# FitSNAP/FitSNAP

Measured on AMD Instinct MI355X. Metric: training rows/sec through A^T A + solve, 1000000 x 128 fp64 in total over the GPUs (strong scaling), higher is better.
Workload: dtype f64

## Files before the change

fitsnap_amd/build.py:

```python
from __future__ import annotations

import hashlib
import os
import shutil
import subprocess
import sys

HERE = os.path.dirname(os.path.abspath(__file__))
CSRC = os.path.join(HERE, "csrc")
LIBDIR = os.path.join(HERE, "_lib")
LIBNAME = "libfsnap_hip.so"
SOURCES = ["fsnap_syrk_quad.hip:0", "fsnap_syrk_quad.hip:1", "fsnap_syrk_quad.hip:2", "fsnap_syrk.hip", "fsnap_syrk_short.hip", "fsnap_rows.hip", "fsnap_chol.hip", "fsnap_trsm.hip", "fsnap_fused.hip", "fsnap_merr.hip", "fsnap_cand.hip", "fsnap_uq.hip", "fsnap_loco.hip", "fsnap_mcmc.hip", "fsnap_capi.cpp", "fsnap_comm.cpp", "fsnap_p2p.cpp",
           "fsnap_rowspace.cpp", "fsnap_rowspace_host.cpp", "fsnap_solve.cpp"]
HEADERS = ["fsnap_kernels.h", "fsnap_device_common.h", "fsnap_ctx.h", "fsnap_rowspace_host.h", "fsnap_condest.h", "fsnap_p2p.h", os.path.join("..", "..", "include", "fsnap_hip.h")]
ARCH = "gfx950"


def lib_path() -> str:
    return os.path.join(LIBDIR, LIBNAME)


def _hipcc() -> str:
    exe = shutil.which("hipcc") or "/opt/rocm/bin/hipcc"
    if not os.path.exists(exe):
        raise RuntimeError("hipcc not found: libfsnap_hip.so cannot be built")
    return exe


def _source_digest() -> str:
    h = hashlib.sha256()
    for name in sorted({s.split(":")[0] for s in SOURCES}) + HEADERS:
        with open(os.path.join(CSRC, name), "rb") as f:
            h.update(f.read())
    return h.hexdigest()


def build_library(force: bool = False, verbose: bool = False) -> str:
    os.makedirs(LIBDIR, exist_ok=True)
    out = lib_path()
    stamp = out + ".sha256"
    digest = _source_digest()
    if not force and os.path.exists(out) and os.path.exists(stamp):
        with open(stamp) as f:
            if f.read().strip() == digest:
                return out
    hipcc = _hipcc()
    objs = []
    common = [f"--offload-arch={ARCH}", "-O3", "-std=c++17", "-fPIC", "-I", os.path.join(HERE, "..", "include")]
    procs = []
    objdir = os.path.join(LIBDIR, "obj")
    os.makedirs(objdir, exist_ok=True)
    hh = hashlib.sha256()
    for name in HEADERS:
        with open(os.path.join(CSRC, name), "rb") as f:
            hh.update(f.read())
    for entry in SOURCES:
        src, _, part = entry.partition(":")
        obj = os.path.join(objdir, os.path.splitext(src)[0] + (f"_{part}" if part else "") + ".o")
        cmd = [hipcc, *common]
        if part:
            cmd += [f"-DFSNAP_QUAD_PART={part}"]
        if src in ("fsnap_capi.cpp", "fsnap_comm.cpp", "fsnap_p2p.cpp", "fsnap_rowspace.cpp"):
            cmd += ["-x", "hip"]
        if src in ("fsnap_solve.cpp", "fsnap_rowspace_host.cpp"):
            cmd = [hipcc, "-x", "c++", "-O3", "-std=c++17", "-fPIC", "-mavx2", "-mfma",
# ... 39 lines not shown
```

fitsnap_amd/csrc/fsnap_capi.cpp:

```cpp
#include <hip/hip_runtime.h>

#include <algorithm>
#include <atomic>
#include <chrono>
#include <cstdarg>
#include <cstdio>
#include <cstdlib>
#include <cstring>
#include <limits>
#include <new>
#include <queue>
#include <string>
#include <thread>
#include <vector>

#include "../../include/fsnap_hip.h"
#include "fsnap_kernels.h"

extern "C" int fsnap_solve_diag_tagged(int kind, double param, int64_t K, const double* G, const double* c, const double* diag,
                                       double* beta, int* rank, double* rcond_est, int upper, const void* owner,
                                       unsigned long long generation);
extern "C" int fsnap_solve_diag_upper(int kind, double param, int64_t K, const double* G, const double* c, const double* diag,
                                      double* beta, int* rank, double* rcond_est);
extern "C" int fsnap_solve_diag(int kind, double param, int64_t K, const double* G, const double* c, const double* diag,
// ... 523 lines not shown
    a.nblocks = g.nblocks;
    a.split = g.split;
    a.chunks_per_wave = g.cpw;
    a.nontemporal = true;
    a.part = (double*)ctx->part.p;
    a.cpart = (double*)ctx->cpart.p;
    a.spart = (double*)ctx->spart.p;
    int ns = -1;
    const double* spart_src = a.spart;
    if (g.fused_pack) {
        a.fused_pack = true;
    } else {
        int npk = 0;
        if ((rc = ensure_wpack(ctx, &npk))) return rc;
        a.wpack = ctx->wpack_override ? ctx->wpack_override : (const double*)ctx->wpack.p;
        spart_src = (const double*)ctx->wpack_spart.p;
        ns = npk;
    }
    hipEvent_t* evs;
    if ((rc = fit_events(ctx, &evs))) return rc;
    if (evs) FSNAP_HIP(hipEventRecord(evs[0], ctx->stream), "hipEventRecord");
    if (g.quad && g.cluster > 1) {
        const size_t need = (size_t)g.nblocks * 4 * sizeof(int);
        if (ctx->quad_flow.bytes < need) {
            if (!ctx->quad_flow.ensure(need)) return ctx->fail(FSNAP_E_NOMEM, "hipMalloc(flow words) failed");
            FSNAP_HIP(hipMemsetAsync(ctx->quad_flow.p, 0, ctx->quad_flow.bytes, ctx->stream), "hipMemset(flow words)");
            ctx->quad_flow_tag = 0;
        }
        ctx->quad_flow_tag += 1u << 20;
        a.flow_words = (int*)ctx->quad_flow.p;
        const int flow = 2 | ((g.cluster == 2 ? 0 : 2) << 2);
        a.flow_tag = (int)(ctx->quad_flow_tag | (unsigned)flow);
    }
    if (g.shortk) FSNAP_HIP(fsnap::launch_syrk_short(a, ctx->stream), "launch fsnap_syrk_short");
    else if (g.quad) FSNAP_HIP(fsnap::launch_syrk_quad(a, ctx->stream), "launch fsnap_syrk_quad");
    else if (g.acc) FSNAP_HIP(fsnap::launch_syrk_acc(a, ctx->stream), "launch fsnap_syrk_acc");
    else FSNAP_HIP(fsnap::launch_syrk_wave_p(a, ctx->stream), "launch fsnap_syrk_wave_p");
    if (evs) FSNAP_HIP(hipEventRecord(evs[1], ctx->stream), "hipEventRecord");
    double* mirror = nullptr;
    if (want_mirror && !device_factor(ctx, ctx->K)) {
        const size_t need = ((size_t)FSNAP_PACKED_LEN(ctx->K) + (size_t)ctx->K) * 8;
        if (ctx->mirror_bytes < need) {
            if (ctx->mirror) (void)hipHostFree(ctx->mirror);
            ctx->mirror = nullptr;
            ctx->mirror_bytes = 0;
            if (hipHostMalloc((void**)&ctx->mirror, need, hipHostMallocCoherent | hipHostMallocMapped) == hipSuccess)
                ctx->mirror_bytes = need;
        }
        if (ctx->mirror && !ctx->mirror_ev && hipEventCreateWithFlags(&ctx->mirror_ev, hipEventDisableTiming) != hipSuccess)
            ctx->mirror_ev = nullptr;
        if (ctx->mirror && ctx->mirror_ev) mirror = ctx->mirror;
    }
    const bool upper_mirror = mirror != nullptr;
    FSNAP_HIP(fsnap::launch_reduce(a.part, a.cpart, spart_src, g.nblocks, cs_per_block, ns, a.K, d_packed, mirror, accumulate,
                                   ctx->stream, upper_mirror),
              "launch fsnap_reduce_partials");
    if (evs) FSNAP_HIP(hipEventRecord(evs[2], ctx->stream), "hipEventRecord");
    if (mirror) {
        FSNAP_HIP(hipEventRecord(ctx->mirror_ev, ctx->stream), "hipEventRecord");
        ctx->mirror_of = d_packed;
        ctx->mirror_K = ctx->K;
        ctx->mirror_upper = upper_mirror;
        ctx->mirror_gen = next_mirror_generation();
    }
    if (evs) ctx->t_syrk = true;
    return FSNAP_OK;
}

}

namespace fsnap {

int wpack_current(fsnap_ctx* ctx) {
    int rc, npk = 0;
    if ((rc = check_rows(ctx)) || (rc = check_weights(ctx))) return rc;
    return ensure_wpack(ctx, &npk);
}

int normal_eq_launch_on(fsnap_ctx* ctx, const double* Q, int64_t ldq, const double* qpack, double* d_packed) {
    const double* const save_A = ctx->dA;
    const int64_t save_lda = ctx->lda;
    ctx->dA = Q;
    ctx->lda = ldq;
    ctx->wpack_override = qpack;
    const int rc = launch_normal_eq(ctx, d_packed);
    ctx->wpack_override = nullptr;
    ctx->dA = save_A;
    ctx->lda = save_lda;
    return rc;
}

}

extern "C" {

int fsnap_version(void) { return 200; }

int fsnap_device_count(int* count) {
    if (!count) return FSNAP_E_ARG;
    int n = 0;
    hipError_t e = hipGetDeviceCount(&n);
    if (e != hipSuccess) {
        g_last_error = std::string("hipGetDeviceCount: ") + hipGetErrorString(e);
        *count = 0;
        return FSNAP_E_HIP;
    }
    *count = n;
    return FSNAP_OK;
}
// ... 86 lines not shown

int fsnap_ctx_set_stream(fsnap_ctx* ctx, void* hip_stream) {
    if (!ctx) return FSNAP_E_ARG;
    FSNAP_HIP(hipStreamSynchronize(ctx->stream), "hipStreamSynchronize");
    ctx->stream = (hipStream_t)hip_stream;
    return FSNAP_OK;
}

int fsnap_ctx_use_own_stream(fsnap_ctx* ctx) {
    if (!ctx) return FSNAP_E_ARG;
    FSNAP_HIP(hipStreamSynchronize(ctx->stream), "hipStreamSynchronize");
    ctx->stream = ctx->own_stream;
    return FSNAP_OK;
}

int fsnap_set_option(fsnap_ctx* ctx, const char* key, int64_t value) {
    if (!ctx || !key) return FSNAP_E_ARG;
    if (!strcmp(key, "device_solve")) {
        if (value < 0 || value > 2) return ctx->fail(FSNAP_E_ARG, "device_solve must be 0 (auto), 1 (always) or 2 (never)");
        ctx->opt_device_solve = (int)value;
    } else if (!strcmp(key, "tiled")) {
        ctx->opt_tiled = value != 0;
    } else if (!strcmp(key, "short")) {
        if (value < -1 || value > 1) return ctx->fail(FSNAP_E_ARG, "short must be -1 (by the row count), 0 (never) or 1 (always)");
        ctx->opt_short = (int)value;
    } else if (!strcmp(key, "timing_every")) {
        if (value < 0 || value > (1 << 20)) return ctx->fail(FSNAP_E_ARG, "timing_every out of range");
        ctx->opt_timing_every = (int)value;
        ctx->timing_phase = 0;
    } else if (!strcmp(key, "repack")) {
        ctx->opt_repack = value != 0;
    } else if (!strcmp(key, "comm_timeout")) {
        if (value < 0 || value > 86400) return ctx->fail(FSNAP_E_ARG, "comm_timeout must be 0 (FSNAP_COMM_TIMEOUT) ... 86400 seconds");
        ctx->opt_comm_timeout = (int)value;
    } else if (!strcmp(key, "chol_reuse")) {
        ctx->opt_chol_reuse = value != 0;
        ctx->chol_factor_of = nullptr;
    } else if (!strcmp(key, "rowspace_reuse_stats")) {
        ctx->opt_rowspace_reuse = value != 0;
    } else if (!strcmp(key, "quad_min_rows")) {
        if (value < -1) return ctx->fail(FSNAP_E_ARG, "quad_min_rows must be >= -1");
        ctx->opt_quad_min_rows = value;
    } else if (!strcmp(key, "reduce_triangle")) {
        if (value < -1 || value > 1) return ctx->fail(FSNAP_E_ARG, "reduce_triangle must be -1 (K >= 256), 0 (never) or 1 (always)");
        ctx->opt_reduce_triangle = (int)value;
    } else if (!strcmp(key, "staged_upload")) {
        if (value < 0 || value > 2) return ctx->fail(FSNAP_E_ARG, "staged_upload must be 0 (pageable copy), 1 (probe) or 2 (double buffer)");
        ctx->opt_staged_upload = (int)value;
    } else if (!strcmp(key, "fused_residual")) {
        if (value < 0 || value > 1) return ctx->fail(FSNAP_E_ARG, "fused_residual must be 0 (two kernels) or 1 (one pass)");
        ctx->opt_fused_residual = (int)value;
    } else if (!strcmp(key, "fused_pack")) {
        ctx->opt_fused_pack = value != 0;
    } else if (!strcmp(key, "nsplit")) {
        if (value < 0 || value > (1 << 24)) return ctx->fail(FSNAP_E_ARG, "nsplit out of range");
        ctx->opt_nsplit = (int)value;
    } else if (!strcmp(key, "nblocks")) {
        if (value < 0 || value > (1 << 24)) return ctx->fail(FSNAP_E_ARG, "nblocks out of range");
        ctx->opt_nblocks = (int)value;
    } else {
        return ctx->fail(FSNAP_E_ARG, "unknown option '%s'", key);
    }
    return FSNAP_OK;
}

int fsnap_upload_rows(fsnap_ctx* ctx, const double* A, int64_t m, int64_t K, int64_t lda, const double* b) {
    if (!ctx) return FSNAP_E_ARG;
    if (!A || !b || m <= 0 || K <= 0 || lda < K) return ctx->fail(FSNAP_E_ARG, "fsnap_upload_rows: bad argument");
    FSNAP_HIP(hipSetDevice(ctx->device), "hipSetDevice");
    const size_t abytes = (size_t)m * K * sizeof(double);
    if (!ctx->ownA.ensure(abytes + 256) || !ctx->ownb.ensure((size_t)m * sizeof(double)))
        return ctx->fail(FSNAP_E_NOMEM, "hipMalloc of %zu bytes for A failed", abytes);
    FSNAP_HIP(hipEventRecord(ctx->ev[3], ctx->stream), "hipEventRecord");
    FSNAP_HIP(hipMemsetAsync((char*)ctx->ownA.p + abytes, 0, 256, ctx->stream), "hipMemsetAsync");
    size_t done_rows = 0;
    int staged = FSNAP_E_STATE;
    const bool fits = (size_t)K * 8 <= ((size_t)16 << 20);
    if (ctx->opt_staged_upload == 2 && abytes >= ((size_t)8 << 20) && fits) {
        staged = staged_rows_h2d(ctx, ctx->ownA.p, A, (size_t)m, (size_t)K * 8, (size_t)lda * 8, 0.0, &done_rows);
        if (staged != FSNAP_OK && staged != FSNAP_E_NOMEM) return staged;
        if (staged != FSNAP_OK) done_rows = 0;
    } else if (ctx->opt_staged_upload == 1 && abytes >= ((size_t)256 << 20) && fits) {
        double rate = 0.0;
        staged = staged_rows_h2d(ctx, ctx->ownA.p, A, (size_t)m, (size_t)K * 8, (size_t)lda * 8, 20.0e9, &done_rows, &rate);
        if (staged != FSNAP_OK && staged != FSNAP_E_NOMEM) return staged;
        if (staged != FSNAP_OK) done_rows = 0;
        ctx->upload_probe_gbps = rate / 1e9;
    }
    const size_t rest = (size_t)m - done_rows;
    if (rest > 0) {
        staged = FSNAP_E_STATE;
        if (lda == K) {
            FSNAP_HIP(hipMemcpyAsync((char*)ctx->ownA.p + done_rows * (size_t)K * 8, A + done_rows * (size_t)lda, rest * (size_t)K * 8,
                                     hipMemcpyHostToDevice, ctx->stream),
                      "hipMemcpy(A)");
        } else {
            FSNAP_HIP(hipMemcpy2DAsync((char*)ctx->ownA.p + done_rows * (size_t)K * 8, (size_t)K * 8, A + done_rows * (size_t)lda,
                                       (size_t)lda * 8, (size_t)K * 8, rest, hipMemcpyHostToDevice, ctx->stream),
                      "hipMemcpy2D(A)");
        }
    }
    ctx->upload_staged = staged == FSNAP_OK;
    FSNAP_HIP(hipMemcpyAsync(ctx->ownb.p, b, (size_t)m * 8, hipMemcpyHostToDevice, ctx->stream), "hipMemcpy(b)");
    FSNAP_HIP(hipEventRecord(ctx->ev[4], ctx->stream), "hipEventRecord");
    FSNAP_HIP(hipStreamSynchronize(ctx->stream), "hipStreamSynchronize");
    ctx->t_upload = true;
// ... 1571 lines not shown
```

fitsnap_amd/csrc/fsnap_ctx.h:

```cpp
#pragma once
#include <hip/hip_runtime.h>

#include <cstdarg>
#include <cstdio>
#include <string>
#include <vector>

#include "../../include/fsnap_hip.h"

namespace fsnap {

constexpr int64_t DEVICE_CHOL_MIN_K = 232;

std::string& library_error();

struct DevBuf {
    void* p = nullptr;
    size_t bytes = 0;
    bool ensure(size_t n) {
        if (n <= bytes && p) return true;
        if (p) (void)hipFree(p);
        p = nullptr;
        bytes = 0;
        if (hipMalloc(&p, n) != hipSuccess) {
// ... 85 lines not shown
    double* pinned = nullptr;
    size_t pinned_bytes = 0;
    double* mirror = nullptr;
    size_t mirror_bytes = 0;
    const double* mirror_of = nullptr;
    int64_t mirror_K = 0;
    unsigned long long mirror_gen = 0;
    bool mirror_upper = false;
    hipEvent_t mirror_ev = nullptr;
    int opt_nblocks = 0;
    int opt_tiled = 0;
    int opt_short = -1;
    int opt_nsplit = 0;
    int opt_device_solve = 0;
    bool tplan_valid = false;
    int64_t tplan_key[4] = {0, 0, 0, 0};
    int tplan[3] = {0, 0, 0};
    int64_t tplan_cps = 0;
    bool t_syrk = false, t_upload = false, t_weight = false, t_predict = false;

    char* wstage[2] = {nullptr, nullptr};
    size_t wstage_bytes[2] = {0, 0};
    hipEvent_t wstage_ev[2] = {nullptr, nullptr};
    int wstage_next = 0;
    const double* chol_factor_of = nullptr;
    int64_t chol_factor_K = 0;
    double chol_factor_alpha = 0.0;
    double chol_factor_rcond = 0.0;
    double chol_factor_piv = 0.0, chol_factor_lam = 0.0;
    std::vector<double> probe_gram;
    int probe_n = 0;
    int h2d_method = -1;
    int h2d_probes = 0;
    double h2d_best[2] = {1.0e30, 1.0e30};
    hipEvent_t h2d_ev = nullptr;
    char* rstage[2] = {nullptr, nullptr};
    hipEvent_t rstage_ev[2] = {nullptr, nullptr};
    bool rstage_busy[2] = {false, false};
    DevBuf wtrain, wrank;
    int64_t ntrain_resident = -1;

    fsnap::Comm* comm = nullptr;
    fsnap::RowSpace* rowspace = nullptr;
    int (*dense_pinv)(void*, int64_t, int64_t, const double*, double, const double*, double*, int*) = nullptr;
    void* dense_pinv_user = nullptr;
    int64_t dense_pinv_token = 0;
    DevBuf commbuf;
    DevBuf tribuf;
    int opt_reduce_triangle = -1;
    int opt_staged_upload = 0;
    double upload_probe_gbps = 0.0;
    bool upload_staged = false;
    int opt_fused_residual = 1;
    int opt_fused_pack = 1;
    int opt_rowspace_reuse = 0;
    int opt_chol_reuse = 1;
    int64_t opt_quad_min_rows = -1;
    int opt_repack = 0;
    int opt_comm_timeout = 0;
    bool comm_broken = false;

    int fail(int code, const char* fmt, ...) {
        char buf[512];
        va_list ap;
        va_start(ap, fmt);
        vsnprintf(buf, sizeof buf, fmt, ap);
        va_end(ap);
        err = buf;
        fsnap::library_error() = buf;
        return code;
    }
    int hipfail(hipError_t e, const char* what) {
        return fail(e == hipErrorOutOfMemory ? FSNAP_E_NOMEM : FSNAP_E_HIP, "%s: %s", what, hipGetErrorString(e));
    }
};


#define FSNAP_HIP(call, what)                                \
    do {                                                     \
        hipError_t _e = (call);                              \
        if (_e != hipSuccess) return ctx->hipfail(_e, what); \
    } while (0)

namespace fsnap {
double comm_timeout_s();
double comm_timeout_s(const fsnap_ctx* ctx);
int wait_stream(fsnap_ctx* ctx, hipEvent_t ev, const char* what);
int allreduce_packed(fsnap_ctx* ctx, double* dp, int64_t K);
bool allreduce_packed_reserve(fsnap_ctx* ctx, int64_t K);
int normal_eq_launch_on(fsnap_ctx* ctx, const double* Q, int64_t ldq, const double* qpack, double* d_packed);
int wpack_current(fsnap_ctx* ctx);
void rowspace_release(fsnap_ctx* ctx);
}
```

fitsnap_amd/csrc/fsnap_kernels.h:

```cpp
#pragma once
#include <hip/hip_runtime.h>
#include <stdint.h>

namespace fsnap {

struct SyrkArgs {
    const double* A;
    int64_t lda;
    const double* b;
    const double* w;
    const unsigned char* mask;
    int64_t m;
    int K;
    int nblocks;
    int split;
    int64_t chunks_per_wave;
    bool nontemporal;
    double* part;
    double* cpart;
    double* spart;
    const double* wpack = nullptr;
    int* flow_words = nullptr;
    int flow_tag = 0;
    bool fused_pack = false;
};

struct TiledArgs {
    const double* A;
    int64_t lda;
    const double* wpack;
    int64_t m;
    int K;
    int NSB;
    int npairs;
    int nsplit;
    int64_t chunks_per_split;
    bool nontemporal;
    double* part;
    double* cpart;
    const double* spart;
    int ns;
};

int syrk_num_blocks(int K);
int syrk_waves_per_simd(int K, int split);
hipError_t launch_syrk_wave_p(const SyrkArgs& a, hipStream_t st);
hipError_t launch_syrk_acc(const SyrkArgs& a, hipStream_t st);
hipError_t launch_syrk_quad(const SyrkArgs& a, hipStream_t st);
int64_t syrk_quad_max_cpg();
int syrk_quad_cluster(int K);
int64_t syrk_acc_max_fused_cpw();
hipError_t launch_syrk_short(const SyrkArgs& a, hipStream_t st);
bool syrk_short_takes(int K);
int syrk_short_phase_rows(int K);
int64_t syrk_wave_p_max_fused_cpw(int K, int wg_per_cu);
hipError_t launch_reduce(const double* part, const double* cpart, const double* spart, int nblocks,
                         int cs_per_block, int ns, int K, double* out, double* mirror, bool accumulate, hipStream_t st,
                         bool upper_mirror = false);
int pack_weights_num_blocks(int64_t m);
hipError_t launch_pack_weights(const double* b, const double* w, const unsigned char* mask, int64_t m, double* wpack,
                               double* spart, hipStream_t st);
hipError_t launch_syrk_tiled(const TiledArgs& a, hipStream_t st);
hipError_t launch_reduce_tiled(const TiledArgs& a, double* out, bool accumulate, hipStream_t st);
hipError_t launch_weight_rows(const double* A, int64_t lda, const double* b, const double* w,
                              const unsigned char* mask, int64_t m, int K, double* aw, int64_t ldaw, double* bw,
                              hipStream_t st);
hipError_t launch_assemble(const double* raw, int64_t raw_ld, int64_t nrows, const int64_t* src_row, const int* kind,
                           const int* frac, const double* dval, const double* truth, const double* weight,
                           const double* fractions, const double* blank2J, int ntypes, int ncoeff, int off, double* A,
                           int64_t lda, double* b, double* w, hipStream_t st);
size_t assemble_row_record_bytes();
hipError_t launch_assemble_bw(const double* raw, int64_t raw_ld, int64_t nrows, const int64_t* src_row, const int* kind,
                              const int* frac, const double* d, const double* truth, const double* weight, int icolref,
                              double* b, double* w, void* recs, hipStream_t st);
hipError_t launch_assemble_syrk(const double* raw, int64_t raw_ld, const void* recs, const double* dval, const double* fractions,
                                const double* blank2J, int ntypes, int ncoeff, int off, const TiledArgs& a, hipStream_t st);
hipError_t launch_mirror_copy(const double* src, int K, double* mirror, hipStream_t st);
hipError_t launch_tri_pack(const double* packed, int K, double* tri, hipStream_t st);
hipError_t launch_tri_unpack(const double* tri, int K, double* packed, hipStream_t st);
size_t chol_large_work_doubles(int n);
hipError_t launch_chol_large(const double* packed, const double* cvec, int n, double alpha, double* work, double* dsc, double* z,
                             double* beta, int* status, double* minpiv, double* host_out, bool clear_status, double* probe_out,
                             hipStream_t st);
constexpr int CHOL_PROBES = 31;
double chol_probe(int row, int p);
hipError_t launch_chol_resolve(const double* d_rhs, int n, double* work, const double* dsc, double* z, double* beta, int* status,
                               const double* minpiv, double* host_out, hipStream_t st);
hipError_t launch_chol_factor(const double* G, int n, double shift, double* work, double* dsc, int* status, double* minpiv,
                              int K16, double* Rout, hipStream_t st);
hipError_t launch_gram_scan(const double* G, int n, double* out, hipStream_t st);
int gemv_num_blocks(int64_t m);
hipError_t launch_gemv_rows(const double* A, int64_t lda, const double* beta, int64_t m, int K, double* preds,
                            const double* b, const double* w, const unsigned char* mask, double* sse_part,
                            double* uout, hipStream_t st, bool uplain = false);
int gemvT_num_blocks(int64_t m);
int residual_num_blocks(int64_t m, int K);
hipError_t launch_residual_rows(const double* A, int64_t lda, const double* beta, int64_t m, int K, const double* b,
                                const double* w, const unsigned char* mask, double* partial, double* sse_part, double* out,
                                hipStream_t st);
hipError_t launch_colsum(const double* partial, int nparts, int ncols, double* out, hipStream_t st);
hipError_t launch_expand_weights(const double* wtrain, const unsigned char* mask, const int* rank, int64_t m, double* w,
                                 hipStream_t st);
int error_stats_num_blocks(int64_t m);
hipError_t launch_error_stats(const double* truth, const double* pred, const double* wgt, const int* cat, int64_t m, int ncat,
                              int pass, const double* means, double* partial, hipStream_t st);
hipError_t launch_gemvT_rows(const double* A, int64_t lda, const double* u, int64_t m, int K, double* partial,
                             double* out, hipStream_t st);

constexpr int MERR_IID = 0, MERR_ABC = 1, MERR_FULL = 2;
constexpr int MERR_ONE_PASS_MAX_K = 288;
int merr_num_blocks(int64_t m, int K);
// ... 68 lines not shown
```

fitsnap_amd/csrc/fsnap_solve.cpp:

```cpp
#include <atomic>
#include <chrono>
#include <cstdio>
#include <cmath>
#include <cstdlib>
#include <cstdint>
#include <cstring>
#include <limits>
#include <thread>
#include <vector>

#include "../../include/fsnap_hip.h"
#include "fsnap_condest.h"

static thread_local double g_cond_info[4] = {0.0, 0.0, 0.0, 0.0};

extern "C" __attribute__((visibility("hidden"))) void fsnap_cond_note(double min_pivot, double lambda_min, int steps, int where) {
    g_cond_info[0] = min_pivot;
    g_cond_info[1] = lambda_min;
    g_cond_info[2] = (double)steps;
    g_cond_info[3] = (double)where;
}

extern "C" int fsnap_cond_info(double* info) {
    if (!info) return FSNAP_E_ARG;
// ... 183 lines not shown
                *(v8du*)(r3) = y30; *(v8du*)(r3 + 8) = y31; *(v8du*)(r3 + 16) = y32; *(v8du*)(r3 + 24) = y33;
            }
        }
        if (cw == 16) {
            for (; i + 4 <= i_end; i += 4) {
                double* r0 = a + (size_t)i * n + c0;
                double* r1 = r0 + n;
                double* r2 = r1 + n;
                double* r3 = r2 + n;
                v8d y00 = *(const v8du*)(r0), y01 = *(const v8du*)(r0 + 8);
                v8d y10 = *(const v8du*)(r1), y11 = *(const v8du*)(r1 + 8);
                v8d y20 = *(const v8du*)(r2), y21 = *(const v8du*)(r2 + 8);
                v8d y30 = *(const v8du*)(r3), y31 = *(const v8du*)(r3 + 8);
                const double* uk = a + (size_t)jb * n;
                for (int k = 0; k < nk; ++k, uk += n) {
                    const v8d u0 = *(const v8du*)(uk + c0), u1 = *(const v8du*)(uk + c0 + 8);
                    const double f0 = uk[i], f1 = uk[i + 1], f2 = uk[i + 2], f3 = uk[i + 3];
                    const v8d b0 = {f0, f0, f0, f0, f0, f0, f0, f0}, b1 = {f1, f1, f1, f1, f1, f1, f1, f1};
                    const v8d b2 = {f2, f2, f2, f2, f2, f2, f2, f2}, b3 = {f3, f3, f3, f3, f3, f3, f3, f3};
                    y00 -= b0 * u0; y01 -= b0 * u1;
                    y10 -= b1 * u0; y11 -= b1 * u1;
                    y20 -= b2 * u0; y21 -= b2 * u1;
                    y30 -= b3 * u0; y31 -= b3 * u1;
                }
                *(v8du*)(r0) = y00; *(v8du*)(r0 + 8) = y01;
                *(v8du*)(r1) = y10; *(v8du*)(r1 + 8) = y11;
                *(v8du*)(r2) = y20; *(v8du*)(r2 + 8) = y21;
                *(v8du*)(r3) = y30; *(v8du*)(r3 + 8) = y31;
            }
        }
        for (; i < i_end; ++i) {
            double* ri = a + (size_t)i * n + c0;
            const double* uk = a + (size_t)jb * n;
            for (int k = 0; k < nk; ++k, uk += n) axpy_neg(ri, uk + c0, uk[i], cw);
        }
    }
}

int chol_upper_rb(double* a, int n, double* min_piv2, int NBK) {
    double mp = std::numeric_limits<double>::infinity();
    for (int jb = 0; jb < n; jb += NBK) {
        const int je = (jb + NBK < n) ? jb + NBK : n;
        const int fail = chol_panel(a, n, jb, je, &mp);
        if (fail >= 0) {
            if (min_piv2) *min_piv2 = mp;
            return fail;
        }
        if (je < n) chol_trailing_chunks(a, n, jb, je, 0, 1);
    }
    if (min_piv2) *min_piv2 = mp;
    return -1;
}

FSNAP_CLONES void chol_solve_inv(const double* u, int n, double* x, double* inv) {
    for (int k = 0; k < n; ++k) inv[k] = 1.0 / u[(size_t)k * n + k];
    for (int k = 0; k < n; ++k) {
        const double* r = u + (size_t)k * n;
        x[k] *= inv[k];
        axpy_neg(x + k + 1, r + k + 1, x[k], n - 1 - k);
    }
    for (int i = n - 1; i >= 0; --i) {
        const double* r = u + (size_t)i * n;
        x[i] = (x[i] - dotv(r + i + 1, x + i + 1, n - 1 - i)) * inv[i];
    }
}
void chol_solve(const double* u, int n, double* x) {
    static thread_local vec inv;
    inv.resize(n);
    chol_solve_inv(u, n, x, inv.data());
}

bool lu_solve(double* a, int n, double* b) {
    std::vector<int> piv(n);
    for (int j = 0; j < n; ++j) {
        int p = j;
        double mx = std::fabs(a[(size_t)j * n + j]);
        for (int i = j + 1; i < n; ++i) {
            double v = std::fabs(a[(size_t)i * n + j]);
            if (v > mx) {
                mx = v;
                p = i;
            }
        }
        if (!(mx > 0.0) || !std::isfinite(mx)) return false;
        if (p != j) {
            for (int k = 0; k < n; ++k) std::swap(a[(size_t)j * n + k], a[(size_t)p * n + k]);
            std::swap(b[j], b[p]);
        }
        const double inv = 1.0 / a[(size_t)j * n + j];
        for (int i = j + 1; i < n; ++i) {
            double f = a[(size_t)i * n + j] * inv;
            if (f == 0.0) continue;
            a[(size_t)i * n + j] = f;
            for (int k = j + 1; k < n; ++k) a[(size_t)i * n + k] -= f * a[(size_t)j * n + k];
            b[i] -= f * b[j];
        }
    }
    for (int i = n - 1; i >= 0; --i) {
        double s = b[i];
        for (int k = i + 1; k < n; ++k) s -= a[(size_t)i * n + k] * b[k];
        b[i] = s / a[(size_t)i * n + i];
    }
    return true;
}

void jacobi_eigh(double* a, int n, double* eval, double* v) {
// ... 188 lines not shown

int chol_upper_rb_mt(double* a, int n, double* min_piv2, int NBK, int nt) {
    struct Shared {
        std::atomic<int> arrived{0};
        std::atomic<int> phase{0};
        std::atomic<int> fail{-1};
        double mp = std::numeric_limits<double>::infinity();
    } sh;
    auto barrier = [&](int& local_phase) {
        ++local_phase;
        if (sh.arrived.fetch_add(1, std::memory_order_acq_rel) + 1 == nt) {
            sh.arrived.store(0, std::memory_order_relaxed);
            sh.phase.store(local_phase, std::memory_order_release);
        } else {
            int spins = 0;
            while (sh.phase.load(std::memory_order_acquire) != local_phase) {
#if defined(__x86_64__)
                __builtin_ia32_pause();
#endif
                if (++spins > 4096) {
                    std::this_thread::yield();
                    spins = 0;
                }
            }
        }
    };
    auto body = [&](int t) {
        int ph = 0;
        for (int jb = 0; jb < n; jb += NBK) {
            const int je = (jb + NBK < n) ? jb + NBK : n;
            if (t == 0) {
                const int f = chol_panel_diag(a, n, jb, je, &sh.mp);
                if (f >= 0) sh.fail.store(f, std::memory_order_relaxed);
            }
            barrier(ph);
            if (sh.fail.load(std::memory_order_relaxed) >= 0) return;
            if (je < n) {
                chol_panel_tails(a, n, jb, je, t, nt);
                barrier(ph);
                chol_trailing_chunks(a, n, jb, je, t, nt);
            }
            barrier(ph);
        }
    };
    std::vector<std::thread> th;
    th.reserve(nt - 1);
    for (int t = 1; t < nt; ++t) th.emplace_back(body, t);
    body(0);
    for (auto& x : th) x.join();
    if (min_piv2) *min_piv2 = sh.mp;
    return sh.fail.load();
}

int fast_chol(double* u, int n, double* mp2) {
    static const int forced = [] {
        const char* e = std::getenv("FSNAP_CHOL_VARIANT");
        return e ? std::atoi(e) : 0;
    }();
    static const int nbk_env = [] {
        const char* e = std::getenv("FSNAP_CHOL_NBK");
        return e ? std::atoi(e) : 0;
    }();
    if (forced == 1) return chol_upper(u, n, mp2);
    if (forced == 2) return chol_upper_blocked(u, n, mp2, 64);
    if (forced == 3 || n >= 48) {
        const int nbk = nbk_env > 0 ? nbk_env : (n <= 256 ? 8 : 32);
        static const int nt_env = [] {
            const char* e = std::getenv("FSNAP_CHOL_THREADS");
            return e ? std::atoi(e) : 0;
        }();
        static const int nt_auto = [] {
            auto quota = [](const char* path, bool v2) -> bool {
                FILE* f = std::fopen(path, "r");
                if (!f) return false;
                char buf[64] = {0};
                const bool got = std::fgets(buf, sizeof buf, f) != nullptr;
                std::fclose(f);
                if (!got) return false;
                return v2 ? std::strncmp(buf, "max", 3) != 0 : std::atol(buf) > 0;
            };
            if (quota("/sys/fs/cgroup/cpu.max", true) || quota("/sys/fs/cgroup/cpu/cpu.cfs_quota_us", false)) return 1;
            const unsigned hc = std::thread::hardware_concurrency();
            return (int)(hc >= 8 ? 8 : (hc > 0 ? hc : 1));
        }();
        int nt = nt_env > 0 ? nt_env : nt_auto;
        if (nt > n / 160) nt = n / 160;
        if (nt > 1) return chol_upper_rb_mt(u, n, mp2, nbk, nt);
        return chol_upper_rb(u, n, mp2, nbk);
    }
    return chol_upper(u, n, mp2);
}

}

namespace {
struct PhaseTimer {
    bool on;
    std::chrono::steady_clock::time_point t0;
    PhaseTimer() : on(std::getenv("FSNAP_SOLVE_TIMING") != nullptr), t0(std::chrono::steady_clock::now()) {}
    void lap(const char* what) {
        if (!on) return;
        const auto t1 = std::chrono::steady_clock::now();
        std::fprintf(stderr, "[fsnap_solve] %-14s %9.1f us\n", what, std::chrono::duration<double, std::micro>(t1 - t0).count());
        t0 = t1;
    }
};
}

extern "C" int fsnap_solve_diag(int kind, double param, int64_t K64, const double* G, const double* c, const double* diag,
                                double* beta, int* rank_out, double* rcond_est);
extern "C" int fsnap_solve_diag_upper(int kind, double param, int64_t K64, const double* G, const double* c, const double* diag,
                                      double* beta, int* rank_out, double* rcond_est);
namespace {
int solve_impl(int kind, double param, int64_t K64, const double* G, const double* c, const double* diag, double* beta,
               int* rank_out, double* rcond_est, bool upper_only, const void* owner = nullptr, unsigned long long generation = 0);
// ... 72 lines not shown
    if (!G || !c || !beta || K64 <= 0 || K64 > (1 << 20)) return FSNAP_E_ARG;
    if (kind < FSNAP_SOLVE_CHOL || kind > FSNAP_SOLVE_RIDGE_INV_PROBE) return FSNAP_E_ARG;
    const bool probe = kind >= FSNAP_SOLVE_LSTSQ_PROBE;
    if (kind == FSNAP_SOLVE_LSTSQ_PROBE) kind = FSNAP_SOLVE_LSTSQ;
    if (kind == FSNAP_SOLVE_RIDGE_PROBE) kind = FSNAP_SOLVE_RIDGE;
    if (kind == FSNAP_SOLVE_RIDGE_INV_PROBE) kind = FSNAP_SOLVE_RIDGE_INV;
    const int K = (int)K64;
    if (!std::isfinite(param)) return FSNAP_NUM_NONFINITE;
    const double alpha = (kind == FSNAP_SOLVE_RIDGE || kind == FSNAP_SOLVE_RIDGE_INV) ? param : 0.0;
    const double eps = std::numeric_limits<double>::epsilon();
    timer.lap("finite check");

    {
        int Kp = (K >= 48 && (K & 15) != 0) ? ((K + 15) & ~15) : K;
        if (Kp >= 384 && (Kp & 127) == 0) Kp += 32;
        static thread_local vec U, dsc, z;
        static thread_local struct { const void* owner; unsigned long long gen; int K; double alpha, mp2, piv, lam; } held = {nullptr, 0, 0, 0.0, 0.0, 0.0, 0.0};
        if (owner && held.owner == owner && held.gen == generation && held.K == K && held.alpha == alpha &&
            U.size() == (size_t)Kp * Kp) {
            bool fin = true;
            for (int i = 0; i < K; ++i) {
                z[i] = c[i] * dsc[i];
                fin = fin && (c[i] - c[i] == 0.0);
            }
            if (fin) {
                for (int i = K; i < Kp; ++i) z[i] = 0.0;
                chol_solve(U.data(), Kp, z.data());
                for (int i = 0; i < K; ++i) beta[i] = z[i] * dsc[i];
                timer.lap("tri solves (factor reused)");
                if (all_finite(beta, K)) {
                    if (rank_out) *rank_out = K;
                    if (rcond_est) *rcond_est = held.mp2;
                    fsnap_cond_note(held.piv, held.lam, 0, 0);
                    return FSNAP_OK;
                }
            }
        }
        held.owner = nullptr;
        U.resize((size_t)Kp * Kp);
        dsc.resize(Kp);
        z.resize(Kp);
        bool ok = true;
        double chk = 0.0;
        for (int i = 0; i < K && ok; ++i) {
            const double g = (diag ? diag[i] : G[(size_t)i * K + i]) + alpha;
            if (!(g > 0.0) || !std::isfinite(g)) ok = false;
            else dsc[i] = 1.0 / std::sqrt(g);
            chk += c[i] * 0.0;
        }
        timer.lap("diag scale");
        if (ok) {
            const v8d zero = {0, 0, 0, 0, 0, 0, 0, 0};
            v8d chk0 = zero, chk1 = zero;
            for (int i = 0; i < K; ++i) {
                const double* gi = G + (size_t)i * K;
                double* ui = U.data() + (size_t)i * Kp;
                const double di = dsc[i];
                const v8d dv = {di, di, di, di, di, di, di, di};
                const int j0 = i & ~7;
                if (i + 2 < K) {
                    const double* gn = G + (size_t)(i + 2) * K;
                    for (int jp = (i + 2) & ~7; jp < K; jp += 8) __builtin_prefetch(gn + jp, 0, 0);
                }
                int j = 0;
                for (; j + 8 <= j0; j += 8) *(v8du*)(ui + j) = zero;
                if (upper_only && j + 8 <= K) {
                    typedef long long v8l __attribute__((vector_size(64)));
                    const v8l lanes = {0, 1, 2, 3, 4, 5, 6, 7};
                    const v8l keep = (lanes + (long long)j) >= (long long)i;
                    const v8d g0 = (v8d)((v8l)(*(const v8du*)(gi + j)) & keep);
                    chk0 += g0 * zero;
                    *(v8du*)(ui + j) = g0 * dv * *(const v8du*)(dsc.data() + j);
                    j += 8;
                }
                for (; j + 16 <= K; j += 16) {
                    const v8d g0 = *(const v8du*)(gi + j), g1 = *(const v8du*)(gi + j + 8);
                    chk0 += g0 * zero;
                    chk1 += g1 * zero;
                    *(v8du*)(ui + j) = g0 * dv * *(const v8du*)(dsc.data() + j);
                    *(v8du*)(ui + j + 8) = g1 * dv * *(const v8du*)(dsc.data() + j + 8);
                }
                for (; j + 8 <= K; j += 8) {
                    const v8d g0 = *(const v8du*)(gi + j);
                    chk0 += g0 * zero;
                    *(v8du*)(ui + j) = g0 * dv * *(const v8du*)(dsc.data() + j);
                }
                for (; j < K; ++j) {
                    const double gij = (upper_only && j < i) ? 0.0 : gi[j];
                    ui[j] = gij * di * dsc[j];
                    chk += gij * 0.0;
                }
                for (; j < Kp; ++j) ui[j] = 0.0;
                ui[i] = (gi[i] + alpha) * di * di;
            }
            for (int i = K; i < Kp; ++i) {
                double* ui = U.data() + (size_t)i * Kp;
                for (int j = 0; j < Kp; ++j) ui[j] = 0.0;
                ui[i] = 1.0;
            }
            const v8d cs = chk0 + chk1;
            chk += ((cs[0] + cs[1]) + (cs[2] + cs[3])) + ((cs[4] + cs[5]) + (cs[6] + cs[7]));
            double mp2 = 0.0;
            timer.lap("scale/build");
            const bool fact_ok = (chk == 0.0) && fast_chol(U.data(), Kp, &mp2) < 0;
            timer.lap("cholesky");
            fsnap::CondEstimate ce;
            bool cond_ok = true;
            if (fact_ok && mp2 > 1.0e-3 && kind == FSNAP_SOLVE_LSTSQ) {
                const double* Up = U.data();
                ce = fsnap::lanczos_lambda_min(Kp, [Up, Kp](double* v) {
                    chol_solve(Up, Kp, v);
                    return true;
                });
                cond_ok = ce.lambda_min > 64.0 * K * eps;
                timer.lap("cond estimate");
            }
            if (fact_ok && mp2 > 1.0e-3 && cond_ok) {
                const double piv = mp2;
                if (ce.steps && ce.lambda_min < mp2) mp2 = ce.lambda_min;
                fsnap_cond_note(piv, ce.lambda_min, ce.steps, 0);
                for (int i = 0; i < K; ++i) z[i] = c[i] * dsc[i];
                for (int i = K; i < Kp; ++i) z[i] = 0.0;
                chol_solve(U.data(), Kp, z.data());
                for (int i = 0; i < K; ++i) beta[i] = z[i] * dsc[i];
                timer.lap("tri solves");
                if (all_finite(beta, K)) {
                    if (rank_out) *rank_out = K;
                    if (rcond_est) *rcond_est = mp2;
                    if (owner) {
                        held.owner = owner;
                        held.gen = generation;
                        held.K = K;
                        held.alpha = alpha;
                        held.mp2 = mp2;
                        held.piv = piv;
                        held.lam = ce.lambda_min;
                    }
                    return FSNAP_OK;
                }
            }
        }
    }

    static thread_local vec Gfull;
    if (upper_only) {
        Gfull.resize((size_t)K * K);
        for (int i = 0; i < K; ++i)
            for (int j = i; j < K; ++j) Gfull[(size_t)i * K + j] = Gfull[(size_t)j * K + i] = G[(size_t)i * K + j];
        G = Gfull.data();
    }
    if (!all_finite(G, (size_t)K * K) || !all_finite(c, K)) return FSNAP_NUM_NONFINITE;
    static thread_local Reduced R;
    R.idx.clear();
    R.idx.reserve(K);
    for (int j = 0; j < K; ++j) {
        const double gjj = G[(size_t)j * K + j] + alpha;
        if (gjj == 0.0 && kind != FSNAP_SOLVE_CHOL && kind != FSNAP_SOLVE_RIDGE_INV) continue;
        R.idx.push_back(j);
// ... 130 lines not shown
```

Measured before the change: 3.064 billion.

## Add row-wise finish kernel for partial reduction and fuse Gram build into Cholesky

Adds a new fsnap_finish_rows kernel, on by default for non-quad SYRK paths, that reduces per-block partials row by row. It writes both triangles of the Gram matrix plus the mirror directly, replacing the previous reduce kernel. Separately, the host solve now builds the scaled matrix U lazily in column chunks interleaved with a right-looking blocked Cholesky, so the fill and the factorization share cache. The costs are more complex indexing, new env-driven paths, and possible differences in summation order and numerics.

Result: slower. 2.965 billion (-3.2%).

```diff
diff --git a/fitsnap_amd/build.py b/fitsnap_amd/build.py
--- a/fitsnap_amd/build.py
+++ b/fitsnap_amd/build.py
@@ -10,7 +10,7 @@
 CSRC = os.path.join(HERE, "csrc")
 LIBDIR = os.path.join(HERE, "_lib")
 LIBNAME = "libfsnap_hip.so"
-SOURCES = ["fsnap_syrk_quad.hip:0", "fsnap_syrk_quad.hip:1", "fsnap_syrk_quad.hip:2", "fsnap_syrk.hip", "fsnap_syrk_short.hip", "fsnap_rows.hip", "fsnap_chol.hip", "fsnap_trsm.hip", "fsnap_fused.hip", "fsnap_merr.hip", "fsnap_cand.hip", "fsnap_uq.hip", "fsnap_loco.hip", "fsnap_mcmc.hip", "fsnap_capi.cpp", "fsnap_comm.cpp", "fsnap_p2p.cpp",
+SOURCES = ["fsnap_syrk_quad.hip:0", "fsnap_syrk_quad.hip:1", "fsnap_syrk_quad.hip:2", "fsnap_syrk.hip", "fsnap_syrk_short.hip", "fsnap_finish.hip", "fsnap_rows.hip", "fsnap_chol.hip", "fsnap_trsm.hip", "fsnap_fused.hip", "fsnap_merr.hip", "fsnap_cand.hip", "fsnap_uq.hip", "fsnap_loco.hip", "fsnap_mcmc.hip", "fsnap_capi.cpp", "fsnap_comm.cpp", "fsnap_p2p.cpp",
            "fsnap_rowspace.cpp", "fsnap_rowspace_host.cpp", "fsnap_solve.cpp"]
 HEADERS = ["fsnap_kernels.h", "fsnap_device_common.h", "fsnap_ctx.h", "fsnap_rowspace_host.h", "fsnap_condest.h", "fsnap_p2p.h", os.path.join("..", "..", "include", "fsnap_hip.h")]
 ARCH = "gfx950"
diff --git a/fitsnap_amd/csrc/fsnap_capi.cpp b/fitsnap_amd/csrc/fsnap_capi.cpp
--- a/fitsnap_amd/csrc/fsnap_capi.cpp
+++ b/fitsnap_amd/csrc/fsnap_capi.cpp
@@ -599,9 +599,14 @@
         if (ctx->mirror && ctx->mirror_ev) mirror = ctx->mirror;
     }
     const bool upper_mirror = mirror != nullptr;
-    FSNAP_HIP(fsnap::launch_reduce(a.part, a.cpart, spart_src, g.nblocks, cs_per_block, ns, a.K, d_packed, mirror, accumulate,
-                                   ctx->stream, upper_mirror),
-              "launch fsnap_reduce_partials");
+    if (!g.quad && ctx->opt_finish)
+        FSNAP_HIP(fsnap::launch_finish(a.part, a.cpart, spart_src, g.nblocks, cs_per_block, ns, a.K, d_packed, mirror, accumulate,
+                                       ctx->stream, upper_mirror),
+                  "launch fsnap_finish");
+    else
+        FSNAP_HIP(fsnap::launch_reduce(a.part, a.cpart, spart_src, g.nblocks, cs_per_block, ns, a.K, d_packed, mirror, accumulate,
+                                       ctx->stream, upper_mirror),
+                  "launch fsnap_reduce_partials");
     if (evs) FSNAP_HIP(hipEventRecord(evs[2], ctx->stream), "hipEventRecord");
     if (mirror) {
         FSNAP_HIP(hipEventRecord(ctx->mirror_ev, ctx->stream), "hipEventRecord");
@@ -794,6 +799,9 @@
         ctx->opt_fused_residual = (int)value;
     } else if (!strcmp(key, "fused_pack")) {
         ctx->opt_fused_pack = value != 0;
+    } else if (!strcmp(key, "finish")) {
+        if (value < 0 || value > 1) return ctx->fail(FSNAP_E_ARG, "finish must be 0 (kernel 2b) or 1 (kernel 2c)");
+        ctx->opt_finish = (int)value;
     } else if (!strcmp(key, "nsplit")) {
         if (value < 0 || value > (1 << 24)) return ctx->fail(FSNAP_E_ARG, "nsplit out of range");
         ctx->opt_nsplit = (int)value;
diff --git a/fitsnap_amd/csrc/fsnap_ctx.h b/fitsnap_amd/csrc/fsnap_ctx.h
--- a/fitsnap_amd/csrc/fsnap_ctx.h
+++ b/fitsnap_amd/csrc/fsnap_ctx.h
@@ -161,6 +161,7 @@
     double upload_probe_gbps = 0.0;
     bool upload_staged = false;
     int opt_fused_residual = 1;
+    int opt_finish = 1;
     int opt_fused_pack = 1;
     int opt_rowspace_reuse = 0;
     int opt_chol_reuse = 1;
diff --git a/fitsnap_amd/csrc/fsnap_finish.hip b/fitsnap_amd/csrc/fsnap_finish.hip
--- /dev/null
+++ b/fitsnap_amd/csrc/fsnap_finish.hip
@@ -0,0 +1,155 @@
+#include "fsnap_device_common.h"
+#include "fsnap_kernels.h"
+
+namespace {
+
+__host__ __device__ constexpr int tri_index(int p, int q, int NB) {
+    return p * NB - (p * (p - 1)) / 2 + (q - p);
+}
+
+__device__ __forceinline__ int tile_off(int ep, int eq) { return (ep >> 2) * 64 + (ep & 3) * 16 + eq; }
+
+__device__ __forceinline__ d2 sum_partials(const double* __restrict__ s, int64_t stride, int np, int slice) {
+    d2 a0 = {0.0, 0.0}, a1 = a0, a2 = a0, a3 = a0;
+    int p = slice;
+    for (; p + 240 < np; p += 256) {
+        d2 x[16];
+#pragma unroll
+        for (int j = 0; j < 16; ++j) x[j] = *reinterpret_cast<const d2*>(s + (int64_t)(p + 16 * j) * stride);
+#pragma unroll
+        for (int j = 0; j < 16; j += 4) {
+            a0 += x[j];
+            a1 += x[j + 1];
+            a2 += x[j + 2];
+            a3 += x[j + 3];
+        }
+    }
+    for (; p < np; p += 16) a0 += *reinterpret_cast<const d2*>(s + (int64_t)p * stride);
+    return (a0 + a1) + (a2 + a3);
+}
+
+}
+
+__global__ __launch_bounds__(256) void fsnap_finish_rows(const double* __restrict__ part, const double* __restrict__ cpart,
+                                                         const double* __restrict__ spart, int nblocks, int cs_per_block,
+                                                         int ns, int NB, int K, double* __restrict__ out,
+                                                         double* __restrict__ mirror, int accumulate, int upper_mirror,
+                                                         int vec) {
+    __shared__ __attribute__((aligned(16))) double red[16][32];
+    const int NTILE = NB * (NB + 1) / 2;
+    const int nG = NTILE * 256, nC = NB * 16;
+    const int NG = (NB + 1) >> 1;
+    const int tid = threadIdx.x, sub = tid & 15, slice = tid >> 4;
+    const int h = sub >> 3, eq0 = 2 * (sub & 7);
+    int b = blockIdx.x;
+    int region = 0, P = 0;
+    for (; P < NG; ++P) {
+        const int rows = K - 32 * P < 32 ? K - 32 * P : 32;
+        const int cnt = rows * (NG - P);
+        if (b < cnt) break;
+        b -= cnt;
+    }
+    int r = 0, Q = 0;
+    if (P < NG) {
+        r = 32 * P + b / (NG - P);
+        Q = P + b % (NG - P);
+    } else if (b < NG) {
+        region = 1;
+        Q = b;
+    } else {
+        region = 2;
+    }
+    const bool single_q = (NB & 1) && Q == NG - 1;
+    const int q = single_q ? NB - 1 : 2 * Q + h;
+    bool active;
+    int o0, j0, j1, np, ncols;
+    bool odd_diag = false, even_diag = false;
+    const double* src;
+    int64_t stride;
+    if (region == 2) {
+        active = sub < 2;
+        o0 = 2 * sub; j0 = o0; j1 = o0 + 1;
+        src = spart; stride = 4; np = ns >= 0 ? ns : nblocks * cs_per_block; ncols = 3;
+    } else {
+        active = !(single_q && h == 1);
+        j0 = single_q ? eq0 : 2 * eq0 + h;
+        j1 = single_q ? eq0 + 1 : j0 + 2;
+        ncols = K - 32 * Q < (single_q ? 16 : 32) ? K - 32 * Q : (single_q ? 16 : 32);
+        if (region == 1) {
+            o0 = q * 16 + eq0;
+            src = cpart; stride = nC; np = nblocks * cs_per_block;
+        } else {
+            const bool single_p = (NB & 1) && P == NG - 1;
+            const int rr = r - 32 * P;
+            const int p = single_p ? NB - 1 : 2 * P + (rr & 1), ep = single_p ? rr : rr >> 1;
+            odd_diag = Q == P && !single_p && (rr & 1);
+            even_diag = Q == P && !single_p && !(rr & 1);
+            active = active && p <= q;
+            o0 = tri_index(p <= q ? p : q, q, NB) * 256 + tile_off(ep, eq0);
+            src = part; stride = nG; np = nblocks;
+        }
+    }
+    if (active) {
+        const d2 sv = sum_partials(src + o0, stride, np, slice);
+        red[slice][j0] = sv.x;
+        red[slice][j1] = sv.y;
+    }
+    __syncthreads();
+    if (tid >= 16) return;
+    const int j = 2 * tid;
+    const bool v0 = j < ncols && !odd_diag, v1 = j + 1 < ncols;
+    if (!v0 && !v1) return;
+    d2 tot = *reinterpret_cast<const d2*>(&red[0][j]);
+#pragma unroll
+    for (int k = 1; k < 16; ++k) tot += *reinterpret_cast<const d2*>(&red[k][j]);
+    const int64_t n = (int64_t)K * K;
+    const int64_t at = region == 0 ? (int64_t)r * K + 32 * Q + j : region == 1 ? n + 32 * Q + j : n + K + j;
+    const bool wide = vec && v0 && v1 && region != 2;
+    if (accumulate) {
+        if (wide) {
+            tot += *reinterpret_cast<const d2*>(out + at);
+        } else {
+            if (v0) tot.x += out[at];
+            if (v1) tot.y += out[at + 1];
+        }
+    }
+    const int c = 32 * Q + j;
+    if (wide) {
+        *reinterpret_cast<d2*>(out + at) = tot;
+        if (mirror) *reinterpret_cast<d2*>(mirror + at) = tot;
+    } else {
+        if (v0) out[at] = tot.x;
+        if (v1) out[at + 1] = tot.y;
+        if (mirror) {
+            if (v0) mirror[at] = tot.x;
+            if (v1 && !(odd_diag && upper_mirror && c + 1 < r)) mirror[at + 1] = tot.y;
+        }
+    }
+    if (region != 0) return;
+    const bool t0 = v0 && Q > P, t1 = v1 && (Q > P || even_diag);
+    if (t0) out[(int64_t)c * K + r] = tot.x;
+    if (t1) out[(int64_t)(c + 1) * K + r] = tot.y;
+    if (mirror) {
+        if (t0 && !upper_mirror) mirror[(int64_t)c * K + r] = tot.x;
+        if (t1 && (!upper_mirror || (even_diag && c + 1 < r))) mirror[(int64_t)(c + 1) * K + r] = tot.y;
+        if (Q == P) {
+            if (v0 && c == r) mirror[n + K + 3 + r] = tot.x;
+            else if (v1 && c + 1 == r) mirror[n + K + 3 + r] = tot.y;
+        }
+    }
+}
+
+namespace fsnap {
+
+hipError_t launch_finish(const double* part, const double* cpart, const double* spart, int nblocks, int cs_per_block,
+                         int ns, int K, double* out, double* mirror, bool accumulate, hipStream_t st, bool upper_mirror) {
+    const int NB = syrk_num_blocks(K), NG = (NB + 1) >> 1;
+    int ngroups = NG + 1;
+    for (int P = 0; P < NG; ++P) ngroups += (K - 32 * P < 32 ? K - 32 * P : 32) * (NG - P);
+    const bool vec = (K & 1) == 0 && (((uintptr_t)out | (uintptr_t)mirror) & 15) == 0;
+    hipLaunchKernelGGL(fsnap_finish_rows, dim3((unsigned)ngroups), dim3(256), 0, st, part, cpart, spart, nblocks, cs_per_block,
+                       ns, NB, K, out, mirror, accumulate ? 1 : 0, upper_mirror ? 1 : 0, vec ? 1 : 0);
+    return hipGetLastError();
+}
+
+}
diff --git a/fitsnap_amd/csrc/fsnap_kernels.h b/fitsnap_amd/csrc/fsnap_kernels.h
--- a/fitsnap_amd/csrc/fsnap_kernels.h
+++ b/fitsnap_amd/csrc/fsnap_kernels.h
@@ -57,6 +57,8 @@
 hipError_t launch_reduce(const double* part, const double* cpart, const double* spart, int nblocks,
                          int cs_per_block, int ns, int K, double* out, double* mirror, bool accumulate, hipStream_t st,
                          bool upper_mirror = false);
+hipError_t launch_finish(const double* part, const double* cpart, const double* spart, int nblocks, int cs_per_block,
+                         int ns, int K, double* out, double* mirror, bool accumulate, hipStream_t st, bool upper_mirror);
 int pack_weights_num_blocks(int64_t m);
 hipError_t launch_pack_weights(const double* b, const double* w, const unsigned char* mask, int64_t m, double* wpack,
                                double* spart, hipStream_t st);
diff --git a/fitsnap_amd/csrc/fsnap_solve.cpp b/fitsnap_amd/csrc/fsnap_solve.cpp
--- a/fitsnap_amd/csrc/fsnap_solve.cpp
+++ b/fitsnap_amd/csrc/fsnap_solve.cpp
@@ -259,6 +259,28 @@
     return -1;
 }
 
+template <class Fill>
+int chol_upper_rb_fill(double* a, int n, double* min_piv2, int NBK, Fill&& fill) {
+    double mp = std::numeric_limits<double>::infinity();
+    const int j1 = NBK < n ? NBK : n;
+    fill(0, j1, 0, n);
+    int fail = chol_panel(a, n, 0, j1, &mp);
+    if (fail < 0) {
+        for (int c0 = (j1 >> 5) << 5; c0 < n; c0 += 32) {
+            const int ce = c0 + 32 < n ? c0 + 32 : n;
+            fill(j1, ce, c0, ce);
+            chol_trailing_chunks(a, n, 0, j1, (c0 >> 5) - (j1 >> 5), n);
+        }
+        for (int jb = j1; jb < n && fail < 0; jb += NBK) {
+            const int je = (jb + NBK < n) ? jb + NBK : n;
+            fail = chol_panel(a, n, jb, je, &mp);
+            if (fail < 0 && je < n) chol_trailing_chunks(a, n, jb, je, 0, 1);
+        }
+    }
+    if (min_piv2) *min_piv2 = mp;
+    return fail;
+}
+
 FSNAP_CLONES void chol_solve_inv(const double* u, int n, double* x, double* inv) {
     for (int k = 0; k < n; ++k) inv[k] = 1.0 / u[(size_t)k * n + k];
     for (int k = 0; k < n; ++k) {
@@ -553,15 +575,21 @@
     return sh.fail.load();
 }
 
+int chol_env(const char* name) {
+    const char* e = std::getenv(name);
+    return e ? std::atoi(e) : 0;
+}
+
+int fast_chol_rb_panel(int n) {
+    static const int forced = chol_env("FSNAP_CHOL_VARIANT"), nbk_env = chol_env("FSNAP_CHOL_NBK");
+    static const int fill_off = chol_env("FSNAP_SOLVE_NO_FILL");
+    if (forced != 0 || fill_off || n < 48 || n >= 320) return 0;
+    return nbk_env > 0 ? nbk_env : (n <= 256 ? 8 : 32);
+}
+
 int fast_chol(double* u, int n, double* mp2) {
-    static const int forced = [] {
-        const char* e = std::getenv("FSNAP_CHOL_VARIANT");
-        return e ? std::atoi(e) : 0;
-    }();
-    static const int nbk_env = [] {
-        const char* e = std::getenv("FSNAP_CHOL_NBK");
-        return e ? std::atoi(e) : 0;
-    }();
+    static const int forced = chol_env("FSNAP_CHOL_VARIANT");
+    static const int nbk_env = chol_env("FSNAP_CHOL_NBK");
     if (forced == 1) return chol_upper(u, n, mp2);
     if (forced == 2) return chol_upper_blocked(u, n, mp2, 64);
     if (forced == 3 || n >= 48) {
@@ -740,58 +768,74 @@
         if (ok) {
             const v8d zero = {0, 0, 0, 0, 0, 0, 0, 0};
             v8d chk0 = zero, chk1 = zero;
-            for (int i = 0; i < K; ++i) {
-                const double* gi = G + (size_t)i * K;
-                double* ui = U.data() + (size_t)i * Kp;
-                const double di = dsc[i];
-                const v8d dv = {di, di, di, di, di, di, di, di};
-                const int j0 = i & ~7;
-                if (i + 2 < K) {
-                    const double* gn = G + (size_t)(i + 2) * K;
-                    for (int jp = (i + 2) & ~7; jp < K; jp += 8) __builtin_prefetch(gn + jp, 0, 0);
+            auto fill = [&](int i0, int i1, int cb, int ce) {
+                const int lim = K < ce ? K : ce;
+                for (int i = i0; i < i1; ++i) {
+                    double* ui = U.data() + (size_t)i * Kp;
+                    if (i >= K) {
+                        for (int j = cb; j < ce; ++j) ui[j] = 0.0;
+                        if (cb <= i && i < ce) ui[i] = 1.0;
+                        continue;
+                    }
+                    const double* gi = G + (size_t)i * K;
+                    const double di = dsc[i];
+                    const v8d dv = {di, di, di, di, di, di, di, di};
+                    const int j0 = i & ~7;
+                    if (i + 2 < K) {
+                        const double* gn = G + (size_t)(i + 2) * K;
+                        const int jn = (i + 2) & ~7;
+                        for (int jp = jn > cb ? jn : cb; jp < lim; jp += 8) __builtin_prefetch(gn + jp, 0, 0);
+                    }
+                    int j = cb;
+                    for (; j + 8 <= j0 && j + 8 <= ce; j += 8) *(v8du*)(ui + j) = zero;
+                    if (upper_only && j == j0 && j + 8 <= lim) {
+                        typedef long long v8l __attribute__((vector_size(64)));
+                        const v8l lanes = {0, 1, 2, 3, 4, 5, 6, 7};
+                        const v8l keep = (lanes + (long long)j) >= (long long)i;
+                        const v8d g0 = (v8d)((v8l)(*(const v8du*)(gi + j)) & keep);
+                        chk0 += g0 * zero;
+                        *(v8du*)(ui + j) = g0 * dv * *(const v8du*)(dsc.data() + j);
+                        j += 8;
+                    }
+                    for (; j + 16 <= lim; j += 16) {
+                        const v8d g0 = *(const v8du*)(gi + j), g1 = *(const v8du*)(gi + j + 8);
+                        chk0 += g0 * zero;
+                        chk1 += g1 * zero;
+                        *(v8du*)(ui + j) = g0 * dv * *(const v8du*)(dsc.data() + j);
+                        *(v8du*)(ui + j + 8) = g1 * dv * *(const v8du*)(dsc.data() + j + 8);
+                    }
+                    for (; j + 8 <= lim; j += 8) {
+                        const v8d g0 = *(const v8du*)(gi + j);
+                        chk0 += g0 * zero;
+                        *(v8du*)(ui + j) = g0 * dv * *(const v8du*)(dsc.data() + j);
+                    }
+                    for (; j < lim; ++j) {
+                        const double gij = (upper_only && j < i) ? 0.0 : gi[j];
+                        ui[j] = gij * di * dsc[j];
+                        chk += gij * 0.0;
+                    }
+                    for (; j < ce; ++j) ui[j] = 0.0;
+                    if (cb <= i && i < ce) ui[i] = (gi[i] + alpha) * di * di;
                 }
-                int j = 0;
-                for (; j + 8 <= j0; j += 8) *(v8du*)(ui + j) = zero;
-                if (upper_only && j + 8 <= K) {
-                    typedef long long v8l __attribute__((vector_size(64)));
-                    const v8l lanes = {0, 1, 2, 3, 4, 5, 6, 7};
-                    const v8l keep = (lanes + (long long)j) >= (long long)i;
-                    const v8d g0 = (v8d)((v8l)(*(const v8du*)(gi + j)) & keep);
-                    chk0 += g0 * zero;
-                    *(v8du*)(ui + j) = g0 * dv * *(const v8du*)(dsc.data() + j);
-                    j += 8;
-                }
-                for (; j + 16 <= K; j += 16) {
-                    const v8d g0 = *(const v8du*)(gi + j), g1 = *(const v8du*)(gi + j + 8);
-                    chk0 += g0 * zero;
-                    chk1 += g1 * zero;
-                    *(v8du*)(ui + j) = g0 * dv * *(const v8du*)(dsc.data() + j);
-                    *(v8du*)(ui + j + 8) = g1 * dv * *(const v8du*)(dsc.data() + j + 8);
-                }
-                for (; j + 8 <= K; j += 8) {
-                    const v8d g0 = *(const v8du*)(gi + j);
-                    chk0 += g0 * zero;
-                    *(v8du*)(ui + j) = g0 * dv * *(const v8du*)(dsc.data() + j);
-                }
-                for (; j < K; ++j) {
-                    const double gij = (upper_only && j < i) ? 0.0 : gi[j];
-                    ui[j] = gij * di * dsc[j];
-                    chk += gij * 0.0;
-                }
-                for (; j < Kp; ++j) ui[j] = 0.0;
-                ui[i] = (gi[i] + alpha) * di * di;
-            }
-            for (int i = K; i < Kp; ++i) {
-                double* ui = U.data() + (size_t)i * Kp;
-                for (int j = 0; j < Kp; ++j) ui[j] = 0.0;
-                ui[i] = 1.0;
-            }
-            const v8d cs = chk0 + chk1;
-            chk += ((cs[0] + cs[1]) + (cs[2] + cs[3])) + ((cs[4] + cs[5]) + (cs[6] + cs[7]));
+            };
+            auto fold_chk = [&] {
+                const v8d cs = chk0 + chk1;
+                chk += ((cs[0] + cs[1]) + (cs[2] + cs[3])) + ((cs[4] + cs[5]) + (cs[6] + cs[7]));
+            };
             double mp2 = 0.0;
-            timer.lap("scale/build");
-            const bool fact_ok = (chk == 0.0) && fast_chol(U.data(), Kp, &mp2) < 0;
-            timer.lap("cholesky");
+            bool fact_ok;
+            if (const int nbk = fast_chol_rb_panel(Kp)) {
+                fact_ok = chol_upper_rb_fill(U.data(), Kp, &mp2, nbk, fill) < 0;
+                fold_chk();
+                fact_ok = fact_ok && chk == 0.0;
+                timer.lap("build+cholesky");
+            } else {
+                fill(0, Kp, 0, Kp);
+                fold_chk();
+                timer.lap("scale/build");
+                fact_ok = (chk == 0.0) && fast_chol(U.data(), Kp, &mp2) < 0;
+                timer.lap("cholesky");
+            }
             fsnap::CondEstimate ce;
             bool cond_ok = true;
             if (fact_ok && mp2 > 1.0e-3 && kind == FSNAP_SOLVE_LSTSQ) {
```
